# michaelriedl/2048-ppo-agent

Hardware: AMD Instinct MI355X
Metric: env-steps/sec at N parallel boards (full PPO loop: rollout with policy in the loop + GAE + update) (higher is better)
Workload: dtype u8 boards / bf16 policy; 1 GPU; 65536 parallel boards per GPU, Transformer policy bf16 (3.96 M params), full PPO iteration (BASELINE.json configs[2]; configs[3] when n_gpus=8); boards_per_gpu=65536, global_boards=65536, train_batch=2048, update_epochs=5, max_samples_per_epoch=300000, max_samples_per_epoch_is=global (each rank draws its 1/N share), as the reference's single subset, max_samples_per_epoch_per_rank=300000, rollout_mode=episodes (reference lock-step semantics), rng_mode=partitionable, parallelism=env-shard x1 + 1 grad all-reduce/minibatch

## Files before the change

2048-ppo-agent_amd/csrc/g2048_rowgemm.hip:

```cpp
#include <hip/hip_runtime.h>
#include <stdint.h>
#include <stdlib.h>

#include <type_traits>

#include "../../include/g2048.h"
#include "g2048_host.h"
#include "g2048_mfma.h"

namespace {

using namespace g2048_mfma;
using namespace g2048_host;

constexpr int RG_N = 256, RG_KC = 128, RG_THREADS = 512, RG_WAVES = 8;
template <int NB> struct RgShape {
    static constexpr int TT = 32 * NB, STAGE = TT * RG_KC * 2, PIECES = TT * (RG_KC / 8) / RG_THREADS, RPW = TT / RG_WAVES, BATCH = RPW / 2;
    static constexpr int LDS = 2 * STAGE + RG_WAVES * 3 * RG_N * 4 + RG_N * 4;
    static_assert(PIECES * RG_THREADS == TT * (RG_KC / 8) && RPW % 2 == 0 && BATCH >= 1, "tile shape");
};

enum { RG_FWD = 0, RG_BWD = 1 };

struct RowGemmArgs {
    const __bf16 *x;
    int64_t ldx;
    const __bf16 *w;
    int64_t w_tile_stride;
    const uint16_t *gh_extra;
    int extra_period;
    const float *bias;
    int64_t T;
    int K, tpw;
    const float *res;
    int64_t res_rs;
    const float *g_x;
    int g_x_period;
    const float *gamma, *beta;
    float *mean, *rstd;
    float *out_f32;
    uint16_t *out_bf16;
    float *partial;
    float eps, inv_keep;
    uint32_t thr, s0, s1;
    const uint64_t *seed_state;
};

template <int CTRL>
__device__ __forceinline__ float dpp_step(float v) {
    return v + __builtin_bit_cast(float, __builtin_amdgcn_update_dpp(0, __builtin_bit_cast(int, v), CTRL, 0xF, 0xF, true));
}
__device__ __forceinline__ float wave_sum_dpp(float v) {
    v = dpp_step<0xB1>(v);
    v = dpp_step<0x4E>(v);
    v = dpp_step<0x141>(v);
    v = dpp_step<0x140>(v);
    const int iv = __builtin_bit_cast(int, v);
    const float r0 = __builtin_bit_cast(float, __builtin_amdgcn_readlane(iv, 0)), r1 = __builtin_bit_cast(float, __builtin_amdgcn_readlane(iv, 16));
    const float r2 = __builtin_bit_cast(float, __builtin_amdgcn_readlane(iv, 32)), r3 = __builtin_bit_cast(float, __builtin_amdgcn_readlane(iv, 48));
    return (r0 + r1) + (r2 + r3);
}

template <int MODE, int NB, int NCH>
__global__ void __launch_bounds__(RG_THREADS, 2)
k_rowgemm(RowGemmArgs A) {
    constexpr int RG_NB = NB, RG_TT = RgShape<NB>::TT, RG_STAGE = RgShape<NB>::STAGE, RG_PIECES = RgShape<NB>::PIECES;
    constexpr int RG_RPW = RgShape<NB>::RPW, RG_BATCH = RgShape<NB>::BATCH;
    extern __shared__ __attribute__((aligned(16))) char smem[];
    const int tid = threadIdx.x, lane = tid & 63, r = lane & 31, h = lane >> 5;
    const int w = __builtin_amdgcn_readfirstlane(tid >> 6);
    float *const red = reinterpret_cast<float *>(smem + 2 * RG_STAGE);
    float *const bias_l = reinterpret_cast<float *>(smem + 2 * RG_STAGE + RG_WAVES * 3 * RG_N * 4);
    uint32_t s0 = A.s0, s1 = A.s1;
    mix_seed_state(A.seed_state, s0, s1);
    const int64_t n_tiles = (A.T + A.tpw - 1) / A.tpw;
    if (tid < RG_N) bias_l[tid] = (MODE == RG_FWD && A.bias) ? A.bias[tid] : 0.f;

    for (int64_t tile = blockIdx.x; tile < n_tiles; tile += gridDim.x) {
        const int64_t tok0 = tile * A.tpw;
        const int n_valid = (int)((A.T - tok0 < A.tpw) ? A.T - tok0 : A.tpw);
        uint32_t goff[RG_PIECES];
        const int row0 = tid >> 4, pc = tid & 15;
#pragma unroll
        for (int j = 0; j < RG_PIECES; ++j) {
            const int row = row0 + 32 * j;
            goff[j] = (uint32_t)((int64_t)(row < n_valid ? row : n_valid - 1) * A.ldx * 2) + 16u * (uint32_t)pc;
        }
        const uint32_t loff0 = (uint32_t)(row0 * (RG_KC * 2) + ((pc ^ (row0 & 15)) << 4));
        const char *const xg = reinterpret_cast<const char *>(A.x + tok0 * A.ldx);
        u32x4 G[3][RG_PIECES];
        unsigned kc = 0;
#define RG_GLOAD(P, ahead)                                                                                                \
    _Pragma("unroll") for (int j = 0; j < RG_PIECES; ++j) G[P][j] =                                                       \
        *reinterpret_cast<const u32x4 *>(xg + goff[j] + (size_t)(kc + (ahead)) * (RG_KC * 2))
#define RG_LSTORE(P, ST)                                                                                                  \
    _Pragma("unroll") for (int j = 0; j < RG_PIECES; ++j)                                                                 \
        *reinterpret_cast<u32x4 *>(smem + (ST) * RG_STAGE + loff0 + j * (32 * RG_KC * 2)) = G[P][j]
        constexpr int WR = 4, NG = 8 * NCH;
        const __bf16 *const wp = A.w + (size_t)w * A.w_tile_stride + lane * 8;
        bf16x8 W[WR];
        const uint32_t brow = (uint32_t)(r * (RG_KC * 2)), bx = (uint32_t)((h ^ (r & 15)) << 4);

        f32x16 acc[RG_NB];
        RG_GLOAD(0, 0);
        if constexpr (NCH > 1) { RG_GLOAD(1, 1); }
        if constexpr (NCH > 2) { RG_GLOAD(2, 2); }
#pragma unroll
        for (int g = 0; g < WR; ++g) W[g] = *reinterpret_cast<const bf16x8 *>(wp + (size_t)g * 512);
        lds_barrier();
#pragma unroll
        for (int b = 0; b < RG_NB; ++b) acc[b] = bias_tile(bias_l, 32 * w, h);
        RG_LSTORE(0, 0);
        lds_barrier();

        const bool norm = A.gamma != nullptr;
        const float4 gm = norm ? reinterpret_cast<const float4 *>(A.gamma)[lane] : make_float4(0.f, 0.f, 0.f, 0.f);
        auto row_tok = [&](int row) -> int64_t { return tok0 + (row < n_valid ? row : n_valid - 1); };
        constexpr bool PIPE = NB <= 3;
        constexpr int BB = RG_BATCH / 2, NBB = RG_RPW / BB;
        static_assert(RG_RPW % BB == 0, "backward batches");
        float4 fv[MODE == RG_FWD ? RG_RPW : 1];
        float4 bx0[2][MODE == RG_BWD ? BB : 1], bg0[2][MODE == RG_BWD ? BB : 1];
        float bmu[2][MODE == RG_BWD ? BB : 1], brs[2][MODE == RG_BWD ? BB : 1];
        auto bwd_load = [&](int k, auto parity) {
            constexpr int P = decltype(parity)::value;
#pragma unroll
            for (int j = 0; j < BB; ++j) {
                const int64_t tok = row_tok(w + RG_WAVES * (k * BB + j));
                bx0[P][j] = reinterpret_cast<const float4 *>(A.res + tok * A.res_rs)[lane];
                bmu[P][j] = A.mean[tok];
                brs[P][j] = A.rstd[tok];
                bg0[P][j] = make_float4(0.f, 0.f, 0.f, 0.f);
                if (A.g_x) {
                    if (A.g_x_period == 1) bg0[P][j] = reinterpret_cast<const float4 *>(A.g_x + tok * RG_N)[lane];
                    else if (tok % A.g_x_period == 0) bg0[P][j] = reinterpret_cast<const float4 *>(A.g_x + (tok / A.g_x_period) * RG_N)[lane];
                }
            }
        };
        auto fwd_load = [&](auto lo_c, auto hi_c) {
#pragma unroll
            for (int j = decltype(lo_c)::value; j < decltype(hi_c)::value; ++j)
                fv[j] = reinterpret_cast<const float4 *>(A.res + row_tok(w + RG_WAVES * j) * A.res_rs)[lane];
        };
        using I0 = std::integral_constant<int, 0>;
        using IB = std::integral_constant<int, RG_BATCH>;
        using IR = std::integral_constant<int, RG_RPW>;
#define RG_FRAG(st, s_) \
    *reinterpret_cast<const bf16x8 *>((st) + brow + ((32u * ((s_) / RG_NB)) ^ bx) + ((s_) % RG_NB) * (32 * RG_KC * 2))
#define RG_CHUNK(c)                                                                                                        \
    if constexpr ((c) < NCH) {                                                                                             \
        if constexpr ((c) == NCH - 1 && PIPE) {        \
            if (MODE == RG_FWD) fwd_load(I0{}, IB{});                                                                      \
            else bwd_load(0, I0{});                                                                                        \
        }                                                                                                                  \
        if constexpr ((c) + 3 < NCH) { RG_GLOAD((c) % 3, 3); }                                                             \
        const char *const st = smem + ((c) & 1) * RG_STAGE;                                                                \
        constexpr int PRE = 3, NS = 8 * RG_NB;     \
        bf16x8 q[PRE];                                                                                                     \
        _Pragma("unroll") for (int s_ = 0; s_ < PRE; ++s_) q[s_] = RG_FRAG(st, s_);                                        \
        _Pragma("unroll") for (int s_ = 0; s_ < NS; ++s_) {                                                                \
            __builtin_amdgcn_sched_barrier(0);                                                                             \
            const int ks = s_ / RG_NB, b = s_ % RG_NB, g = 8 * (c) + ks;                                                   \
            acc[b] = mfma(W[g % WR], q[s_ % PRE], acc[b]);                                                                 \
            if (s_ + PRE < NS) q[s_ % PRE] = RG_FRAG(st, s_ + PRE);                                                        \
            if (b == RG_NB - 1 && g + WR < NG) W[g % WR] = *reinterpret_cast<const bf16x8 *>(wp + (size_t)(kc * 8 + ks + WR) * 512); \
        }                                                                                                                  \
        __builtin_amdgcn_sched_barrier(0);                                                                                 \
        if constexpr ((c) + 1 < NCH) { RG_LSTORE(((c) + 1) % 3, ((c) + 1) & 1); }                                          \
        kc += 1;                                                                                                           \
        asm volatile("" : "+s"(kc));                                                                                       \
        lds_barrier();                                                                                                     \
    }
        RG_CHUNK(0) RG_CHUNK(1) RG_CHUNK(2) RG_CHUNK(3) RG_CHUNK(4) RG_CHUNK(5) RG_CHUNK(6) RG_CHUNK(7)
#undef RG_CHUNK
#undef RG_FRAG
#undef RG_GLOAD
#undef RG_LSTORE

#pragma unroll
        for (int b = 0; b < RG_NB; ++b) {
            const int trow = 32 * b + r;
#pragma unroll
            for (int g = 0; g < 4; ++g) {
                const uint32_t lo = f2bf(acc[b][4 * g + 0]) | (f2bf(acc[b][4 * g + 1]) << 16);
                const uint32_t hi = f2bf(acc[b][4 * g + 2]) | (f2bf(acc[b][4 * g + 3]) << 16);
                *reinterpret_cast<uint2 *>(smem + trow * 512 + (((4 * w + g) ^ (trow & 31)) << 4) + 8 * h) = make_uint2(lo, hi);
            }
        }
        lds_barrier();
        if (MODE == RG_FWD) {
            if (PIPE) fwd_load(IB{}, IR{});
            else fwd_load(I0{}, IR{});
        }
        auto tile_row = [&](int row) -> uint2 {
            return *reinterpret_cast<const uint2 *>(smem + row * 512 + ((((lane >> 1) ^ (row & 31))) << 4) + 8 * (lane & 1));
        };
        if (MODE == RG_FWD) {
            const float4 bt = norm ? reinterpret_cast<const float4 *>(A.beta)[lane] : make_float4(0.f, 0.f, 0.f, 0.f);
#pragma unroll
            for (int j0 = 0; j0 < RG_RPW; j0 += RG_BATCH) {
                if (w + RG_WAVES * j0 >= n_valid) break;
                float4 v[RG_BATCH];
                float s[RG_BATCH];
#pragma unroll
                for (int j = 0; j < RG_BATCH; ++j) {
                    const int row = w + RG_WAVES * (j0 + j), rowc = row < n_valid ? row : n_valid - 1;
                    const int64_t tok = tok0 + rowc;
                    const uint2 ab = tile_row(rowc);
                    float av[4] = {bf2f(ab.x & 0xFFFFu), bf2f(ab.x >> 16), bf2f(ab.y & 0xFFFFu), bf2f(ab.y >> 16)};
                    if (A.thr) {
                        const uint64_t base = (uint64_t)tok * RG_N + 4 * lane;
#pragma unroll
                        for (int q = 0; q < 4; ++q) av[q] = keep_elem(s0, s1, A.thr, base + q) ? av[q] * A.inv_keep : 0.0f;
                    }
                    v[j] = fv[j0 + j];
                    v[j].x += av[0]; v[j].y += av[1]; v[j].z += av[2]; v[j].w += av[3];
                    if (row < n_valid) reinterpret_cast<float4 *>(A.out_f32 + tok * RG_N)[lane] = v[j];
                    s[j] = v[j].x + v[j].y + v[j].z + v[j].w;
                }
#pragma unroll
                for (int j = 0; j < RG_BATCH; ++j) s[j] = wave_sum_dpp(s[j]);
                float mean[RG_BATCH];
#pragma unroll
                for (int j = 0; j < RG_BATCH; ++j) {
                    mean[j] = s[j] * (1.0f / RG_N);
                    v[j].x -= mean[j]; v[j].y -= mean[j]; v[j].z -= mean[j]; v[j].w -= mean[j];
                    s[j] = v[j].x * v[j].x + v[j].y * v[j].y + v[j].z * v[j].z + v[j].w * v[j].w;
                }
#pragma unroll
                for (int j = 0; j < RG_BATCH; ++j) s[j] = wave_sum_dpp(s[j]);
#pragma unroll
                for (int j = 0; j < RG_BATCH; ++j) {
                    const int row = w + RG_WAVES * (j0 + j);
                    const int64_t tok = tok0 + row;
                    const float rstd = rsqrtf(s[j] * (1.0f / RG_N) + A.eps);
                    const uint32_t lo = f2bf(v[j].x * rstd * gm.x + bt.x) | (f2bf(v[j].y * rstd * gm.y + bt.y) << 16);
                    const uint32_t hi = f2bf(v[j].z * rstd * gm.z + bt.z) | (f2bf(v[j].w * rstd * gm.w + bt.w) << 16);
                    if (row < n_valid) {
                        reinterpret_cast<uint2 *>(A.out_bf16 + tok * RG_N)[lane] = make_uint2(lo, hi);
                        if (lane == 0) {
                            A.mean[tok] = mean[j];
                            A.rstd[tok] = rstd;
                        }
                    }
                }
            }
        } else {
            float dg[4] = {0, 0, 0, 0}, db[4] = {0, 0, 0, 0}, dsum[4] = {0, 0, 0, 0};
            const float gg[4] = {gm.x, gm.y, gm.z, gm.w};
            auto bwd_batch = [&](int k, auto parity) {
                constexpr int P = decltype(parity)::value;
                if (PIPE && k + 1 < NBB && w + RG_WAVES * (k + 1) * BB < n_valid) bwd_load(k + 1, std::integral_constant<int, P ^ 1>{});
                float xh[BB][4], dxh[BB][4], c1[BB], c2[BB];
#pragma unroll
                for (int j = 0; j < BB; ++j) {
                    const int row = w + RG_WAVES * (k * BB + j), rowc = row < n_valid ? row : n_valid - 1;
                    const float ok = row < n_valid ? 1.f : 0.f;
                    const uint2 gb = tile_row(rowc);
                    float gh[4] = {bf2f(gb.x & 0xFFFFu), bf2f(gb.x >> 16), bf2f(gb.y & 0xFFFFu), bf2f(gb.y >> 16)};
                    if (A.gh_extra) {
                        const int64_t tk = tok0 + rowc;
                        if (tk % A.extra_period == 0) {
                            const uint2 eb = reinterpret_cast<const uint2 *>(A.gh_extra + (tk / A.extra_period) * RG_N)[lane];
                            gh[0] = bf2f(f2bf(gh[0] + bf2f(eb.x & 0xFFFFu))); gh[1] = bf2f(f2bf(gh[1] + bf2f(eb.x >> 16)));
                            gh[2] = bf2f(f2bf(gh[2] + bf2f(eb.y & 0xFFFFu))); gh[3] = bf2f(f2bf(gh[3] + bf2f(eb.y >> 16)));
                        }
                    }
                    const float xs[4] = {bx0[P][j].x, bx0[P][j].y, bx0[P][j].z, bx0[P][j].w};
                    c1[j] = c2[j] = 0.f;
#pragma unroll
                    for (int q = 0; q < 4; ++q) {
                        xh[j][q] = (xs[q] - bmu[P][j]) * brs[P][j];
                        dxh[j][q] = gh[q] * gg[q];
                        c1[j] += dxh[j][q];
                        c2[j] += dxh[j][q] * xh[j][q];
                        dg[q] += ok * (gh[q] * xh[j][q]);
                        db[q] += ok * gh[q];
                    }
                }
#pragma unroll
                for (int j = 0; j < BB; ++j) {
                    c1[j] = wave_sum_dpp(c1[j]);
                    c2[j] = wave_sum_dpp(c2[j]);
                }
#pragma unroll
                for (int j = 0; j < BB; ++j) {
                    const int row = w + RG_WAVES * (k * BB + j);
                    const bool ok = row < n_valid;
                    const int64_t tok = tok0 + (ok ? row : n_valid - 1);
                    float o[4] = {bg0[P][j].x, bg0[P][j].y, bg0[P][j].z, bg0[P][j].w};
                    const float m1 = c1[j] * (1.0f / RG_N), m2 = c2[j] * (1.0f / RG_N);
#pragma unroll
                    for (int q = 0; q < 4; ++q) o[q] += brs[P][j] * (dxh[j][q] - m1 - xh[j][q] * m2);
                    if (ok) reinterpret_cast<float4 *>(A.out_f32 + tok * RG_N)[lane] = make_float4(o[0], o[1], o[2], o[3]);
                    if (A.out_bf16) {
                        if (A.thr) {
                            const uint64_t base = (uint64_t)tok * RG_N + 4 * lane;
#pragma unroll
                            for (int q = 0; q < 4; ++q) o[q] = keep_elem(s0, s1, A.thr, base + q) ? o[q] * A.inv_keep : 0.0f;
                        }
                        uint32_t bq[4];
#pragma unroll
                        for (int q = 0; q < 4; ++q) {
                            bq[q] = f2bf(o[q]);
                            dsum[q] += ok ? bf2f(bq[q]) : 0.f;
                        }
                        if (ok) reinterpret_cast<uint2 *>(A.out_bf16 + tok * RG_N)[lane] = make_uint2(bq[0] | (bq[1] << 16), bq[2] | (bq[3] << 16));
                    }
                }
            };
            if (PIPE) {
#pragma unroll
                for (int k = 0; k < NBB; k += 2) {
                    if (w + RG_WAVES * k * BB < n_valid) bwd_batch(k, std::integral_constant<int, 0>{});
                    if (k + 1 < NBB && w + RG_WAVES * (k + 1) * BB < n_valid) bwd_batch(k + 1, std::integral_constant<int, 1>{});
                }
            } else {
#pragma unroll 1
                for (int k = 0; k < NBB; ++k) {
                    if (w + RG_WAVES * k * BB >= n_valid) break;
                    bwd_load(k, std::integral_constant<int, 0>{});
                    bwd_batch(k, std::integral_constant<int, 0>{});
                }
            }
#pragma unroll
            for (int q = 0; q < 4; ++q) {
                red[(w * 3 + 0) * RG_N + 4 * lane + q] = dg[q];
                red[(w * 3 + 1) * RG_N + 4 * lane + q] = db[q];
                red[(w * 3 + 2) * RG_N + 4 * lane + q] = dsum[q];
            }
            lds_barrier();
            for (int c = tid; c < 3 * RG_N; c += RG_THREADS) {
                float s = 0.f;
#pragma unroll
                for (int ww = 0; ww < RG_WAVES; ++ww) s += red[ww * 3 * RG_N + c];
                float *dst = A.partial + (int64_t)blockIdx.x * 3 * RG_N + c;
                *dst = (tile == (int64_t)blockIdx.x) ? s : *dst + s;
            }
        }
    }
}

inline int rg_tpw(int64_t T, int *nb) {
    const char *e = getenv("G2048_RG_TWO_TILES");
    const bool two = e && e[0] == '1';
    int64_t t = (T + 255) / 256;
    if (two) t = (T + 511) / 512;
    if (t <= 96 && (two || t <= 48)) {
        *nb = 3;
        return (int)(t < 32 ? 32 : t);
    }
    *nb = 5;
    return (int)(t > 160 ? 160 : t);
}

template <int MODE, int NB, int NCH>
int rg_launch3(RowGemmArgs &A, unsigned grid, hipStream_t stream) {
    const void *fn = reinterpret_cast<const void *>(k_rowgemm<MODE, NB, NCH>);
    constexpr int lds = RgShape<NB>::LDS;
    if (const int rc = allow_dynamic_lds(fn, lds)) return rc;
    hipLaunchKernelGGL((k_rowgemm<MODE, NB, NCH>), dim3(grid), dim3(RG_THREADS), lds, stream, A);
    return launch_status();
}
template <int MODE, int NB>
int rg_launch2(RowGemmArgs &A, unsigned grid, hipStream_t stream) {
    switch (A.K / RG_KC) {
        case 2: return rg_launch3<MODE, NB, 2>(A, grid, stream);
        case 4: return rg_launch3<MODE, NB, 4>(A, grid, stream);
        case 6: return rg_launch3<MODE, NB, 6>(A, grid, stream);
        case 8: return rg_launch3<MODE, NB, 8>(A, grid, stream);
        default: return G2048_EINVAL;
    }
}
template <int MODE>
int rg_launch(RowGemmArgs &A, hipStream_t stream) {
    int nb = 5;
    A.tpw = rg_tpw(A.T, &nb);
    const int64_t tiles = (A.T + A.tpw - 1) / A.tpw;
    const unsigned grid = (unsigned)(tiles < 256 ? tiles : 256);
    return nb == 3 ? rg_launch2<MODE, 3>(A, grid, stream) : rg_launch2<MODE, 5>(A, grid, stream);
}

inline bool rg_gemm_ok(const void *x, int64_t ldx, const void *w, int64_t T, int K) {
    return x && w && T > 0 && K >= 256 && K % 256 == 0 && K <= 1024 && ldx >= K && !(ldx & 7) && aligned16(x, w) &&
           (int64_t)160 * ldx * 2 < (1ll << 31);
}

}

extern "C" int64_t g2048_linear_add_ln_bwd_partial_rows(int64_t T) {
    if (T <= 0) return 0;
    int nb;
    const int tpw = rg_tpw(T, &nb);
    const int64_t tiles = (T + tpw - 1) / tpw;
    return tiles < 256 ? tiles : 256;
}

extern "C" int g2048_linear_add_ln_fwd(const void *u, int64_t ldu, const void *w_packed, const float *bias, int K, const float *x,
                                       int64_t x_row_stride, const float *gamma, const float *beta, float *x_new, void *h, float *mean,
                                       float *rstd, int64_t T, float eps, float p_drop, uint64_t seed, const uint64_t *seed_state,
                                       void *stream) {
    if (!rg_gemm_ok(u, ldu, w_packed, T, K) || !x || !gamma || !beta || !x_new || !h || !mean || !rstd || !(p_drop >= 0.f && p_drop < 1.f) ||
        (x_row_stride & 3) || !aligned16(x, gamma, beta, x_new, bias) ||
        ((uintptr_t)h & 7))
        return G2048_EINVAL;
    RowGemmArgs A{};
    A.x = (const __bf16 *)u; A.ldx = ldu; A.w = (const __bf16 *)w_packed; A.bias = bias; A.T = T; A.K = K;
    A.w_tile_stride = (int64_t)(K >> 4) * 512; A.extra_period = 1;
    A.res = x; A.res_rs = x_row_stride; A.gamma = gamma; A.beta = beta; A.mean = mean; A.rstd = rstd; A.out_f32 = x_new;
    A.out_bf16 = (uint16_t *)h; A.eps = eps; A.inv_keep = 1.0f / (1.0f - p_drop); A.thr = (uint32_t)(p_drop * 16777216.0f);
    A.s0 = (uint32_t)seed; A.s1 = (uint32_t)(seed >> 32); A.seed_state = seed_state; A.g_x_period = 1;
    return rg_launch<RG_FWD>(A, (hipStream_t)stream);
}

extern "C" int g2048_linear_add_ln_bwd(const void *dy, int64_t lddy, const void *wt_packed, int64_t wt_tile_stride, int K,
                                       const float *x_norm, int64_t x_row_stride, const float *g_x, int g_x_period, const void *g_h_extra,
                                       int extra_period, const float *mean, const float *rstd, const float *gamma, float *dx, void *da,
                                       float *partial, int64_t T, float p_drop, uint64_t seed, const uint64_t *seed_state, void *stream) {
    if (wt_tile_stride == 0) wt_tile_stride = (int64_t)(K >> 4) * 512;
    if (wt_tile_stride < (int64_t)(K >> 4) * 512 || (wt_tile_stride & 7) || (g_h_extra && extra_period < 1) || ((uintptr_t)g_h_extra & 7))
        return G2048_EINVAL;
    if (!rg_gemm_ok(dy, lddy, wt_packed, T, K) || !x_norm || !mean || !rstd || !gamma || !dx || !partial || g_x_period < 1 ||
        !(p_drop >= 0.f && p_drop < 1.f) || (x_row_stride & 3) ||
        !aligned16(x_norm, g_x, gamma, dx) || ((uintptr_t)da & 7) || ((uintptr_t)partial & 3))
        return G2048_EINVAL;
    if ((g_x && T % g_x_period != 0) || (g_h_extra && T % extra_period != 0)) return G2048_EINVAL;
    RowGemmArgs A{};
    A.x = (const __bf16 *)dy; A.ldx = lddy; A.w = (const __bf16 *)wt_packed; A.T = T; A.K = K;
    A.w_tile_stride = wt_tile_stride; A.gh_extra = (const uint16_t *)g_h_extra; A.extra_period = extra_period < 1 ? 1 : extra_period;
    A.res = x_norm; A.res_rs = x_row_stride; A.g_x = g_x; A.g_x_period = g_x_period; A.gamma = gamma;
    A.mean = const_cast<float *>(mean); A.rstd = const_cast<float *>(rstd); A.out_f32 = dx; A.out_bf16 = (uint16_t *)da;
    A.partial = partial; A.inv_keep = 1.0f / (1.0f - p_drop); A.thr = da ? (uint32_t)(p_drop * 16777216.0f) : 0u;
    A.s0 = (uint32_t)seed; A.s1 = (uint32_t)(seed >> 32); A.seed_state = seed_state;
    return rg_launch<RG_BWD>(A, (hipStream_t)stream);
}
```

Baseline: 3.939 million env-steps/sec.

## Use buffer loads and split residual-row prefetch in row-GEMM LN kernel

Replaces global pointer loads of activations, weights and residual rows with raw buffer loads through per-tile resource descriptors, which gives scalar offsets and hardware bounds clamping. In the backward pass, mean/rstd and periodic g_x offsets are loaded once per lane and broadcast with readlane instead of per-row scalar loads. For larger NB in forward mode, residual-row and gamma prefetches are split into two requests issued inside the MFMA loop so their latency hides behind compute. It also adds optional timestamp instrumentation and an env-selected serial fallback, plus stride validation, which raise code complexity and register pressure.

```diff
diff --git a/2048-ppo-agent_amd/csrc/g2048_rowgemm.hip b/2048-ppo-agent_amd/csrc/g2048_rowgemm.hip
--- a/2048-ppo-agent_amd/csrc/g2048_rowgemm.hip
+++ b/2048-ppo-agent_amd/csrc/g2048_rowgemm.hip
@@ -61,24 +61,59 @@
     return (r0 + r1) + (r2 + r3);
 }
 
-template <int MODE, int NB, int NCH>
+typedef __amdgpu_buffer_rsrc_t rsrc_t;
+__device__ __forceinline__ rsrc_t rg_rsrc(const void *p, uint32_t bytes) {
+    return __builtin_amdgcn_make_buffer_rsrc(const_cast<void *>(p), 0, (int)bytes, 0x00020000);
+}
+template <class V>
+__device__ __forceinline__ V rg_load16(rsrc_t rs, uint32_t lane_off, uint32_t scalar_off) {
+    return __builtin_bit_cast(V, __builtin_amdgcn_raw_buffer_load_b128(rs, (int)lane_off, (int)scalar_off, 0));
+}
+
+#ifdef G2048_RG_STAMPS
+constexpr int RG_PHASES = 8;
+__device__ unsigned long long g_rg_stamps[2][RG_PHASES];
+struct RgStampSite {
+    __device__ __forceinline__ static bool on(int lane, int w) { return lane == 0 && (w == 0 || w == 7) && blockIdx.x % 16 == 0; }
+    __device__ __forceinline__ static unsigned long long *table(int w) { return g_rg_stamps[w == 0 ? 0 : 1]; }
+};
+#define RG_STAMP(k) stamps.mark(k)
+#define RG_TOUCH(v) asm volatile("" ::"v"(v))
+#define RG_DRAIN() asm volatile("s_waitcnt vmcnt(0)" ::: "memory")
+#else
+#define RG_STAMP(k)
+#define RG_TOUCH(v)
+#define RG_DRAIN()
+#endif
+enum { RG_PH_FIRST_CHUNK, RG_PH_KLOOP, RG_PH_STAGE, RG_PH_WAIT_FIRST, RG_PH_ROWS, RG_PH_WAIT_LATER, RG_PH_DRAIN, RG_PH_PARTIAL };
+
+template <int MODE, int NB, int NCH, bool SERIAL>
 __global__ void __launch_bounds__(RG_THREADS, 2)
 k_rowgemm(RowGemmArgs A) {
     constexpr int RG_NB = NB, RG_TT = RgShape<NB>::TT, RG_STAGE = RgShape<NB>::STAGE, RG_PIECES = RgShape<NB>::PIECES;
     constexpr int RG_RPW = RgShape<NB>::RPW, RG_BATCH = RgShape<NB>::BATCH;
     extern __shared__ __attribute__((aligned(16))) char smem[];
-    const int tid = threadIdx.x, lane = tid & 63, r = lane & 31, h = lane >> 5;
-    const int w = __builtin_amdgcn_readfirstlane(tid >> 6);
+    const int tid0 = threadIdx.x;
+    const int w = __builtin_amdgcn_readfirstlane(tid0 >> 6);
     float *const red = reinterpret_cast<float *>(smem + 2 * RG_STAGE);
     float *const bias_l = reinterpret_cast<float *>(smem + 2 * RG_STAGE + RG_WAVES * 3 * RG_N * 4);
     uint32_t s0 = A.s0, s1 = A.s1;
     mix_seed_state(A.seed_state, s0, s1);
     const int64_t n_tiles = (A.T + A.tpw - 1) / A.tpw;
-    if (tid < RG_N) bias_l[tid] = (MODE == RG_FWD && A.bias) ? A.bias[tid] : 0.f;
+    if (tid0 < RG_N) bias_l[tid0] = (MODE == RG_FWD && A.bias) ? A.bias[tid0] : 0.f;
+#ifdef G2048_RG_STAMPS
+    Stamps<RG_PHASES, RgStampSite> stamps;
+    stamps.start();
+#endif
+    const uint32_t res_rs4 = (uint32_t)(A.res_rs * 4);
 
     for (int64_t tile = blockIdx.x; tile < n_tiles; tile += gridDim.x) {
         const int64_t tok0 = tile * A.tpw;
         const int n_valid = (int)((A.T - tok0 < A.tpw) ? A.T - tok0 : A.tpw);
+        int tid = tid0;
+        asm volatile("" : "+v"(tid));
+        const int lane = tid & 63, r = lane & 31, h = lane >> 5;
+        const uint32_t l16 = 16u * (uint32_t)lane;
         uint32_t goff[RG_PIECES];
         const int row0 = tid >> 4, pc = tid & 15;
 #pragma unroll
@@ -87,17 +122,39 @@
             goff[j] = (uint32_t)((int64_t)(row < n_valid ? row : n_valid - 1) * A.ldx * 2) + 16u * (uint32_t)pc;
         }
         const uint32_t loff0 = (uint32_t)(row0 * (RG_KC * 2) + ((pc ^ (row0 & 15)) << 4));
-        const char *const xg = reinterpret_cast<const char *>(A.x + tok0 * A.ldx);
+        const rsrc_t xr = rg_rsrc(A.x + tok0 * A.ldx, (uint32_t)(((int64_t)(n_valid - 1) * A.ldx + A.K) * 2));
+        const rsrc_t wr = rg_rsrc(A.w + (size_t)w * A.w_tile_stride, (uint32_t)(A.K >> 4) * 1024u);
+        const rsrc_t rr = rg_rsrc(A.res + tok0 * A.res_rs, (uint32_t)(((int64_t)(n_valid - 1) * A.res_rs + RG_N) * 4));
+        constexpr uint32_t RG_NONE = 0xFFFFFFFFu;
+        float vmu = 0.f, vrs = 0.f;
+        uint32_t vgo = RG_NONE, veo = RG_NONE;
+        rsrc_t gxr = rg_rsrc(A.res, 0), exr = rg_rsrc(A.res, 0);
+        const rsrc_t nullr = rg_rsrc(A.res, 0);
+        if (MODE == RG_BWD) {
+            const int mrow = w + RG_WAVES * (lane < RgShape<NB>::RPW ? lane : 0);
+            const uint32_t mrowc = (uint32_t)(mrow < n_valid ? mrow : n_valid - 1);
+            vmu = A.mean[tok0 + mrowc];
+            vrs = A.rstd[tok0 + mrowc];
+            auto periodic = [&](const void *base, int period, uint32_t row_bytes, uint32_t &voff) -> rsrc_t {
+                if (!base) return nullr;
+                const uint32_t per = (uint32_t)period, m0 = (uint32_t)(tok0 % period), q0 = m0 ? 1u : 0u;
+                const uint32_t rows = (m0 + (uint32_t)n_valid - 1u) / per + 1u - q0;
+                const uint32_t t = m0 + mrowc, q = t / per;
+                voff = t == q * per ? (q - q0) * row_bytes : RG_NONE;
+                return rg_rsrc(reinterpret_cast<const char *>(base) + (tok0 / period + q0) * row_bytes, rows * row_bytes);
+            };
+            gxr = periodic(A.g_x, A.g_x_period, RG_N * 4, vgo);
+            exr = periodic(A.gh_extra, A.extra_period, RG_N * 2, veo);
+        }
+        auto row_lane = [&](uint32_t v, int idx) -> uint32_t { return (uint32_t)__builtin_amdgcn_readlane((int)v, idx); };
         u32x4 G[3][RG_PIECES];
         unsigned kc = 0;
 #define RG_GLOAD(P, ahead)                                                                                                \
-    _Pragma("unroll") for (int j = 0; j < RG_PIECES; ++j) G[P][j] =                                                       \
-        *reinterpret_cast<const u32x4 *>(xg + goff[j] + (size_t)(kc + (ahead)) * (RG_KC * 2))
+    _Pragma("unroll") for (int j = 0; j < RG_PIECES; ++j) G[P][j] = rg_load16<u32x4>(xr, goff[j], (kc + (ahead)) * (RG_KC * 2))
 #define RG_LSTORE(P, ST)                                                                                                  \
     _Pragma("unroll") for (int j = 0; j < RG_PIECES; ++j)                                                                 \
         *reinterpret_cast<u32x4 *>(smem + (ST) * RG_STAGE + loff0 + j * (32 * RG_KC * 2)) = G[P][j]
         constexpr int WR = 4, NG = 8 * NCH;
-        const __bf16 *const wp = A.w + (size_t)w * A.w_tile_stride + lane * 8;
         bf16x8 W[WR];
         const uint32_t brow = (uint32_t)(r * (RG_KC * 2)), bx = (uint32_t)((h ^ (r & 15)) << 4);
 
@@ -106,53 +163,53 @@
         if constexpr (NCH > 1) { RG_GLOAD(1, 1); }
         if constexpr (NCH > 2) { RG_GLOAD(2, 2); }
 #pragma unroll
-        for (int g = 0; g < WR; ++g) W[g] = *reinterpret_cast<const bf16x8 *>(wp + (size_t)g * 512);
+        for (int g = 0; g < WR; ++g) W[g] = rg_load16<bf16x8>(wr, l16, g * 1024u);
         lds_barrier();
 #pragma unroll
         for (int b = 0; b < RG_NB; ++b) acc[b] = bias_tile(bias_l, 32 * w, h);
         RG_LSTORE(0, 0);
         lds_barrier();
+        RG_STAMP(RG_PH_FIRST_CHUNK);
 
         const bool norm = A.gamma != nullptr;
-        const float4 gm = norm ? reinterpret_cast<const float4 *>(A.gamma)[lane] : make_float4(0.f, 0.f, 0.f, 0.f);
-        auto row_tok = [&](int row) -> int64_t { return tok0 + (row < n_valid ? row : n_valid - 1); };
-        constexpr bool PIPE = NB <= 3;
+        constexpr bool GM_LATE = NB > 3 && !SERIAL && MODE == RG_FWD;
+        float4 gm = make_float4(0.f, 0.f, 0.f, 0.f);
+        if (!GM_LATE && norm) gm = reinterpret_cast<const float4 *>(A.gamma)[lane];
+        constexpr bool PIPE = NB <= 3 || (!SERIAL && MODE == RG_FWD);
+        constexpr bool TWO_REQ = NB > 3 && PIPE;
+        constexpr int ROWREQ = NB <= 3 ? -1 : 4 * NB - 1, REQ_C0 = NCH >= 2 ? NCH - 2 : 0;
         constexpr int BB = RG_BATCH / 2, NBB = RG_RPW / BB;
         static_assert(RG_RPW % BB == 0, "backward batches");
-        float4 fv[MODE == RG_FWD ? RG_RPW : 1];
-        float4 bx0[2][MODE == RG_BWD ? BB : 1], bg0[2][MODE == RG_BWD ? BB : 1];
-        float bmu[2][MODE == RG_BWD ? BB : 1], brs[2][MODE == RG_BWD ? BB : 1];
+        f32x4 fv[MODE == RG_FWD ? RG_RPW : 1];
+        f32x4 bx0[2][MODE == RG_BWD ? BB : 1], bg0[2][MODE == RG_BWD ? BB : 1];
         auto bwd_load = [&](int k, auto parity) {
             constexpr int P = decltype(parity)::value;
 #pragma unroll
             for (int j = 0; j < BB; ++j) {
-                const int64_t tok = row_tok(w + RG_WAVES * (k * BB + j));
-                bx0[P][j] = reinterpret_cast<const float4 *>(A.res + tok * A.res_rs)[lane];
-                bmu[P][j] = A.mean[tok];
-                brs[P][j] = A.rstd[tok];
-                bg0[P][j] = make_float4(0.f, 0.f, 0.f, 0.f);
-                if (A.g_x) {
-                    if (A.g_x_period == 1) bg0[P][j] = reinterpret_cast<const float4 *>(A.g_x + tok * RG_N)[lane];
-                    else if (tok % A.g_x_period == 0) bg0[P][j] = reinterpret_cast<const float4 *>(A.g_x + (tok / A.g_x_period) * RG_N)[lane];
-                }
+                const int row = w + RG_WAVES * (k * BB + j);
+                const uint32_t rowc = (uint32_t)(row < n_valid ? row : n_valid - 1);
+                bx0[P][j] = rg_load16<f32x4>(rr, l16, rowc * res_rs4);
+                const uint32_t go = row_lane(vgo, k * BB + j);
+                bg0[P][j] = rg_load16<f32x4>(go != RG_NONE ? gxr : nullr, l16, go != RG_NONE ? go : 0u);
             }
         };
         auto fwd_load = [&](auto lo_c, auto hi_c) {
 #pragma unroll
-            for (int j = decltype(lo_c)::value; j < decltype(hi_c)::value; ++j)
-                fv[j] = reinterpret_cast<const float4 *>(A.res + row_tok(w + RG_WAVES * j) * A.res_rs)[lane];
+            for (int j = decltype(lo_c)::value; j < decltype(hi_c)::value; ++j) {
+                const int row = w + RG_WAVES * j;
+                fv[j] = rg_load16<f32x4>(rr, l16, (uint32_t)(row < n_valid ? row : n_valid - 1) * res_rs4);
+            }
         };
-        using I0 = std::integral_constant<int, 0>;
-        using IB = std::integral_constant<int, RG_BATCH>;
-        using IR = std::integral_constant<int, RG_RPW>;
+        auto first_rows = [&]() {
+            if (GM_LATE && norm) gm = __builtin_bit_cast(float4, rg_load16<f32x4>(rg_rsrc(A.gamma, RG_N * 4), l16, 0u));
+            if (MODE == RG_FWD) fwd_load(std::integral_constant<int, 0>{}, std::integral_constant<int, RG_BATCH>{});
+            else bwd_load(0, std::integral_constant<int, 0>{});
+        };
 #define RG_FRAG(st, s_) \
     *reinterpret_cast<const bf16x8 *>((st) + brow + ((32u * ((s_) / RG_NB)) ^ bx) + ((s_) % RG_NB) * (32 * RG_KC * 2))
 #define RG_CHUNK(c)                                                                                                        \
     if constexpr ((c) < NCH) {                                                                                             \
-        if constexpr ((c) == NCH - 1 && PIPE) {        \
-            if (MODE == RG_FWD) fwd_load(I0{}, IB{});                                                                      \
-            else bwd_load(0, I0{});                                                                                        \
-        }                                                                                                                  \
+        if constexpr ((c) == NCH - 1 && PIPE && ROWREQ < 0) { first_rows(); }            \
         if constexpr ((c) + 3 < NCH) { RG_GLOAD((c) % 3, 3); }                                                             \
         const char *const st = smem + ((c) & 1) * RG_STAGE;                                                                \
         constexpr int PRE = 3, NS = 8 * RG_NB;     \
@@ -163,7 +220,10 @@
             const int ks = s_ / RG_NB, b = s_ % RG_NB, g = 8 * (c) + ks;                                                   \
             acc[b] = mfma(W[g % WR], q[s_ % PRE], acc[b]);                                                                 \
             if (s_ + PRE < NS) q[s_ % PRE] = RG_FRAG(st, s_ + PRE);                                                        \
-            if (b == RG_NB - 1 && g + WR < NG) W[g % WR] = *reinterpret_cast<const bf16x8 *>(wp + (size_t)(kc * 8 + ks + WR) * 512); \
+            if (b == RG_NB - 1 && g + WR < NG) W[g % WR] = rg_load16<bf16x8>(wr, l16, (kc * 8 + ks + WR) * 1024u);         \
+            if (TWO_REQ && (c) == REQ_C0 && s_ == ROWREQ) first_rows();                                                    \
+            if (TWO_REQ && (c) == NCH - 1 && s_ == ROWREQ)                                                                 \
+                fwd_load(std::integral_constant<int, RG_BATCH>{}, std::integral_constant<int, RG_RPW>{});                  \
         }                                                                                                                  \
         __builtin_amdgcn_sched_barrier(0);                                                                                 \
         if constexpr ((c) + 1 < NCH) { RG_LSTORE(((c) + 1) % 3, ((c) + 1) & 1); }                                          \
@@ -172,6 +232,7 @@
         lds_barrier();                                                                                                     \
     }
         RG_CHUNK(0) RG_CHUNK(1) RG_CHUNK(2) RG_CHUNK(3) RG_CHUNK(4) RG_CHUNK(5) RG_CHUNK(6) RG_CHUNK(7)
+        RG_STAMP(RG_PH_KLOOP);
 #undef RG_CHUNK
 #undef RG_FRAG
 #undef RG_GLOAD
@@ -188,34 +249,42 @@
             }
         }
         lds_barrier();
+        RG_STAMP(RG_PH_STAGE);
         if (MODE == RG_FWD) {
-            if (PIPE) fwd_load(IB{}, IR{});
-            else fwd_load(I0{}, IR{});
+            if (!TWO_REQ) fwd_load(std::integral_constant<int, PIPE ? RG_BATCH : 0>{}, std::integral_constant<int, RG_RPW>{});
+            RG_TOUCH(fv[RG_BATCH - 1].w);
+            RG_STAMP(RG_PH_WAIT_FIRST);
         }
+        int le = lane, we = w;
+        asm volatile("" : "+v"(le), "+s"(we));
         auto tile_row = [&](int row) -> uint2 {
-            return *reinterpret_cast<const uint2 *>(smem + row * 512 + ((((lane >> 1) ^ (row & 31))) << 4) + 8 * (lane & 1));
+            return *reinterpret_cast<const uint2 *>(smem + row * 512 + ((((le >> 1) ^ (row & 31))) << 4) + 8 * (le & 1));
         };
         if (MODE == RG_FWD) {
-            const float4 bt = norm ? reinterpret_cast<const float4 *>(A.beta)[lane] : make_float4(0.f, 0.f, 0.f, 0.f);
+            const float4 bt = norm ? reinterpret_cast<const float4 *>(A.beta)[le] : make_float4(0.f, 0.f, 0.f, 0.f);
 #pragma unroll
             for (int j0 = 0; j0 < RG_RPW; j0 += RG_BATCH) {
-                if (w + RG_WAVES * j0 >= n_valid) break;
-                float4 v[RG_BATCH];
+                if (we + RG_WAVES * j0 >= n_valid) break;
+                if (j0 > 0) {
+                    RG_TOUCH(fv[RG_RPW - 1].w);
+                    RG_STAMP(RG_PH_WAIT_LATER);
+                }
+                f32x4 v[RG_BATCH];
                 float s[RG_BATCH];
 #pragma unroll
                 for (int j = 0; j < RG_BATCH; ++j) {
-                    const int row = w + RG_WAVES * (j0 + j), rowc = row < n_valid ? row : n_valid - 1;
+                    const int row = we + RG_WAVES * (j0 + j), rowc = row < n_valid ? row : n_valid - 1;
                     const int64_t tok = tok0 + rowc;
                     const uint2 ab = tile_row(rowc);
                     float av[4] = {bf2f(ab.x & 0xFFFFu), bf2f(ab.x >> 16), bf2f(ab.y & 0xFFFFu), bf2f(ab.y >> 16)};
                     if (A.thr) {
-                        const uint64_t base = (uint64_t)tok * RG_N + 4 * lane;
+                        const uint64_t base = (uint64_t)tok * RG_N + 4 * le;
 #pragma unroll
                         for (int q = 0; q < 4; ++q) av[q] = keep_elem(s0, s1, A.thr, base + q) ? av[q] * A.inv_keep : 0.0f;
                     }
                     v[j] = fv[j0 + j];
                     v[j].x += av[0]; v[j].y += av[1]; v[j].z += av[2]; v[j].w += av[3];
-                    if (row < n_valid) reinterpret_cast<float4 *>(A.out_f32 + tok * RG_N)[lane] = v[j];
+                    if (row < n_valid) reinterpret_cast<f32x4 *>(A.out_f32 + tok * RG_N)[le] = v[j];
                     s[j] = v[j].x + v[j].y + v[j].z + v[j].w;
                 }
 #pragma unroll
@@ -231,46 +300,54 @@
                 for (int j = 0; j < RG_BATCH; ++j) s[j] = wave_sum_dpp(s[j]);
 #pragma unroll
                 for (int j = 0; j < RG_BATCH; ++j) {
-                    const int row = w + RG_WAVES * (j0 + j);
+                    const int row = we + RG_WAVES * (j0 + j);
                     const int64_t tok = tok0 + row;
                     const float rstd = rsqrtf(s[j] * (1.0f / RG_N) + A.eps);
                     const uint32_t lo = f2bf(v[j].x * rstd * gm.x + bt.x) | (f2bf(v[j].y * rstd * gm.y + bt.y) << 16);
                     const uint32_t hi = f2bf(v[j].z * rstd * gm.z + bt.z) | (f2bf(v[j].w * rstd * gm.w + bt.w) << 16);
                     if (row < n_valid) {
-                        reinterpret_cast<uint2 *>(A.out_bf16 + tok * RG_N)[lane] = make_uint2(lo, hi);
-                        if (lane == 0) {
+                        reinterpret_cast<uint2 *>(A.out_bf16 + tok * RG_N)[le] = make_uint2(lo, hi);
+                        if (le == 0) {
                             A.mean[tok] = mean[j];
                             A.rstd[tok] = rstd;
                         }
                     }
                 }
-            }
+                RG_STAMP(RG_PH_ROWS);
+            }
+            RG_DRAIN();
+            RG_STAMP(RG_PH_DRAIN);
         } else {
             float dg[4] = {0, 0, 0, 0}, db[4] = {0, 0, 0, 0}, dsum[4] = {0, 0, 0, 0};
             const float gg[4] = {gm.x, gm.y, gm.z, gm.w};
             auto bwd_batch = [&](int k, auto parity) {
                 constexpr int P = decltype(parity)::value;
-                if (PIPE && k + 1 < NBB && w + RG_WAVES * (k + 1) * BB < n_valid) bwd_load(k + 1, std::integral_constant<int, P ^ 1>{});
-                float xh[BB][4], dxh[BB][4], c1[BB], c2[BB];
+                if (PIPE && k + 1 < NBB && we + RG_WAVES * (k + 1) * BB < n_valid) bwd_load(k + 1, std::integral_constant<int, P ^ 1>{});
+                RG_TOUCH(bx0[P][BB - 1].w);
+                RG_TOUCH(bg0[P][BB - 1].w);
+                RG_STAMP(k == 0 ? RG_PH_WAIT_FIRST : RG_PH_WAIT_LATER);
+                float xh[BB][4], dxh[BB][4], c1[BB], c2[BB], mu[BB], rs[BB];
 #pragma unroll
                 for (int j = 0; j < BB; ++j) {
-                    const int row = w + RG_WAVES * (k * BB + j), rowc = row < n_valid ? row : n_valid - 1;
+                    const int row = we + RG_WAVES * (k * BB + j), rowc = row < n_valid ? row : n_valid - 1;
                     const float ok = row < n_valid ? 1.f : 0.f;
                     const uint2 gb = tile_row(rowc);
                     float gh[4] = {bf2f(gb.x & 0xFFFFu), bf2f(gb.x >> 16), bf2f(gb.y & 0xFFFFu), bf2f(gb.y >> 16)};
                     if (A.gh_extra) {
-                        const int64_t tk = tok0 + rowc;
-                        if (tk % A.extra_period == 0) {
-                            const uint2 eb = reinterpret_cast<const uint2 *>(A.gh_extra + (tk / A.extra_period) * RG_N)[lane];
+                        const uint32_t eo = row_lane(veo, k * BB + j);
+                        if (eo != RG_NONE) {
+                            const uint2 eb = __builtin_bit_cast(uint2, __builtin_amdgcn_raw_buffer_load_b64(exr, (int)(8u * (uint32_t)le), (int)eo, 0));
                             gh[0] = bf2f(f2bf(gh[0] + bf2f(eb.x & 0xFFFFu))); gh[1] = bf2f(f2bf(gh[1] + bf2f(eb.x >> 16)));
                             gh[2] = bf2f(f2bf(gh[2] + bf2f(eb.y & 0xFFFFu))); gh[3] = bf2f(f2bf(gh[3] + bf2f(eb.y >> 16)));
                         }
                     }
                     const float xs[4] = {bx0[P][j].x, bx0[P][j].y, bx0[P][j].z, bx0[P][j].w};
                     c1[j] = c2[j] = 0.f;
+                    mu[j] = __builtin_bit_cast(float, row_lane(__builtin_bit_cast(uint32_t, vmu), k * BB + j));
+                    rs[j] = __builtin_bit_cast(float, row_lane(__builtin_bit_cast(uint32_t, vrs), k * BB + j));
 #pragma unroll
                     for (int q = 0; q < 4; ++q) {
-                        xh[j][q] = (xs[q] - bmu[P][j]) * brs[P][j];
+                        xh[j][q] = (xs[q] - mu[j]) * rs[j];
                         dxh[j][q] = gh[q] * gg[q];
                         c1[j] += dxh[j][q];
                         c2[j] += dxh[j][q] * xh[j][q];
@@ -285,17 +362,17 @@
                 }
 #pragma unroll
                 for (int j = 0; j < BB; ++j) {
-                    const int row = w + RG_WAVES * (k * BB + j);
+                    const int row = we + RG_WAVES * (k * BB + j);
                     const bool ok = row < n_valid;
                     const int64_t tok = tok0 + (ok ? row : n_valid - 1);
                     float o[4] = {bg0[P][j].x, bg0[P][j].y, bg0[P][j].z, bg0[P][j].w};
                     const float m1 = c1[j] * (1.0f / RG_N), m2 = c2[j] * (1.0f / RG_N);
 #pragma unroll
-                    for (int q = 0; q < 4; ++q) o[q] += brs[P][j] * (dxh[j][q] - m1 - xh[j][q] * m2);
-                    if (ok) reinterpret_cast<float4 *>(A.out_f32 + tok * RG_N)[lane] = make_float4(o[0], o[1], o[2], o[3]);
+                    for (int q = 0; q < 4; ++q) o[q] += rs[j] * (dxh[j][q] - m1 - xh[j][q] * m2);
+                    if (ok) reinterpret_cast<float4 *>(A.out_f32 + tok * RG_N)[le] = make_float4(o[0], o[1], o[2], o[3]);
                     if (A.out_bf16) {
                         if (A.thr) {
-                            const uint64_t base = (uint64_t)tok * RG_N + 4 * lane;
+                            const uint64_t base = (uint64_t)tok * RG_N + 4 * le;
 #pragma unroll
                             for (int q = 0; q < 4; ++q) o[q] = keep_elem(s0, s1, A.thr, base + q) ? o[q] * A.inv_keep : 0.0f;
                         }
@@ -305,40 +382,52 @@
                             bq[q] = f2bf(o[q]);
                             dsum[q] += ok ? bf2f(bq[q]) : 0.f;
                         }
-                        if (ok) reinterpret_cast<uint2 *>(A.out_bf16 + tok * RG_N)[lane] = make_uint2(bq[0] | (bq[1] << 16), bq[2] | (bq[3] << 16));
+                        if (ok) reinterpret_cast<uint2 *>(A.out_bf16 + tok * RG_N)[le] = make_uint2(bq[0] | (bq[1] << 16), bq[2] | (bq[3] << 16));
                     }
                 }
+                RG_STAMP(RG_PH_ROWS);
             };
             if (PIPE) {
 #pragma unroll
                 for (int k = 0; k < NBB; k += 2) {
-                    if (w + RG_WAVES * k * BB < n_valid) bwd_batch(k, std::integral_constant<int, 0>{});
-                    if (k + 1 < NBB && w + RG_WAVES * (k + 1) * BB < n_valid) bwd_batch(k + 1, std::integral_constant<int, 1>{});
+                    if (we + RG_WAVES * k * BB < n_valid) bwd_batch(k, std::integral_constant<int, 0>{});
+                    if (k + 1 < NBB && we + RG_WAVES * (k + 1) * BB < n_valid) bwd_batch(k + 1, std::integral_constant<int, 1>{});
                 }
             } else {
 #pragma unroll 1
                 for (int k = 0; k < NBB; ++k) {
-                    if (w + RG_WAVES * k * BB >= n_valid) break;
+                    if (we + RG_WAVES * k * BB >= n_valid) break;
                     bwd_load(k, std::integral_constant<int, 0>{});
                     bwd_batch(k, std::integral_constant<int, 0>{});
                 }
             }
+            RG_DRAIN();
+            RG_STAMP(RG_PH_DRAIN);
 #pragma unroll
             for (int q = 0; q < 4; ++q) {
-                red[(w * 3 + 0) * RG_N + 4 * lane + q] = dg[q];
-                red[(w * 3 + 1) * RG_N + 4 * lane + q] = db[q];
-                red[(w * 3 + 2) * RG_N + 4 * lane + q] = dsum[q];
+                red[(we * 3 + 0) * RG_N + 4 * le + q] = dg[q];
+                red[(we * 3 + 1) * RG_N + 4 * le + q] = db[q];
+                red[(we * 3 + 2) * RG_N + 4 * le + q] = dsum[q];
             }
             lds_barrier();
-            for (int c = tid; c < 3 * RG_N; c += RG_THREADS) {
+            for (int c = 64 * we + le; c < 3 * RG_N; c += RG_THREADS) {
                 float s = 0.f;
 #pragma unroll
                 for (int ww = 0; ww < RG_WAVES; ++ww) s += red[ww * 3 * RG_N + c];
                 float *dst = A.partial + (int64_t)blockIdx.x * 3 * RG_N + c;
                 *dst = (tile == (int64_t)blockIdx.x) ? s : *dst + s;
             }
+            RG_STAMP(RG_PH_PARTIAL);
         }
     }
+#ifdef G2048_RG_STAMPS
+    stamps.flush(tid0 & 63, w);
+#endif
+}
+
+inline bool rg_serial_rows() {
+    const char *e = getenv("G2048_RG_SERIAL_ROWS");
+    return e && e[0] == '1';
 }
 
 inline int rg_tpw(int64_t T, int *nb) {
@@ -354,13 +443,19 @@
     return (int)(t > 160 ? 160 : t);
 }
 
+template <int MODE, int NB, int NCH, bool SERIAL>
+int rg_launch4(RowGemmArgs &A, unsigned grid, hipStream_t stream) {
+    const void *fn = reinterpret_cast<const void *>(k_rowgemm<MODE, NB, NCH, SERIAL>);
+    constexpr int lds = RgShape<NB>::LDS;
+    if (const int rc = allow_dynamic_lds(fn, lds)) return rc;
+    hipLaunchKernelGGL((k_rowgemm<MODE, NB, NCH, SERIAL>), dim3(grid), dim3(RG_THREADS), lds, stream, A);
+    return launch_status();
+}
 template <int MODE, int NB, int NCH>
 int rg_launch3(RowGemmArgs &A, unsigned grid, hipStream_t stream) {
-    const void *fn = reinterpret_cast<const void *>(k_rowgemm<MODE, NB, NCH>);
-    constexpr int lds = RgShape<NB>::LDS;
-    if (const int rc = allow_dynamic_lds(fn, lds)) return rc;
-    hipLaunchKernelGGL((k_rowgemm<MODE, NB, NCH>), dim3(grid), dim3(RG_THREADS), lds, stream, A);
-    return launch_status();
+    constexpr bool HAS_ARM = NB > 3 && MODE == RG_FWD;
+    if (HAS_ARM && rg_serial_rows()) return rg_launch4<MODE, NB, NCH, HAS_ARM>(A, grid, stream);
+    return rg_launch4<MODE, NB, NCH, false>(A, grid, stream);
 }
 template <int MODE, int NB>
 int rg_launch2(RowGemmArgs &A, unsigned grid, hipStream_t stream) {
@@ -385,6 +480,7 @@
     return x && w && T > 0 && K >= 256 && K % 256 == 0 && K <= 1024 && ldx >= K && !(ldx & 7) && aligned16(x, w) &&
            (int64_t)160 * ldx * 2 < (1ll << 31);
 }
+inline bool rg_res_ok(int64_t row_stride) { return row_stride >= RG_N && (int64_t)160 * row_stride * 4 < (1ll << 31); }
 
 }
 
@@ -401,7 +497,7 @@
                                        float *rstd, int64_t T, float eps, float p_drop, uint64_t seed, const uint64_t *seed_state,
                                        void *stream) {
     if (!rg_gemm_ok(u, ldu, w_packed, T, K) || !x || !gamma || !beta || !x_new || !h || !mean || !rstd || !(p_drop >= 0.f && p_drop < 1.f) ||
-        (x_row_stride & 3) || !aligned16(x, gamma, beta, x_new, bias) ||
+        (x_row_stride & 3) || !rg_res_ok(x_row_stride) || !aligned16(x, gamma, beta, x_new, bias) ||
         ((uintptr_t)h & 7))
         return G2048_EINVAL;
     RowGemmArgs A{};
@@ -421,7 +517,7 @@
     if (wt_tile_stride < (int64_t)(K >> 4) * 512 || (wt_tile_stride & 7) || (g_h_extra && extra_period < 1) || ((uintptr_t)g_h_extra & 7))
         return G2048_EINVAL;
     if (!rg_gemm_ok(dy, lddy, wt_packed, T, K) || !x_norm || !mean || !rstd || !gamma || !dx || !partial || g_x_period < 1 ||
-        !(p_drop >= 0.f && p_drop < 1.f) || (x_row_stride & 3) ||
+        !(p_drop >= 0.f && p_drop < 1.f) || (x_row_stride & 3) || !rg_res_ok(x_row_stride) ||
         !aligned16(x_norm, g_x, gamma, dx) || ((uintptr_t)da & 7) || ((uintptr_t)partial & 3))
         return G2048_EINVAL;
     if ((g_x && T % g_x_period != 0) || (g_h_extra && T % extra_period != 0)) return G2048_EINVAL;
@@ -434,3 +530,14 @@
     A.s0 = (uint32_t)seed; A.s1 = (uint32_t)(seed >> 32); A.seed_state = seed_state;
     return rg_launch<RG_BWD>(A, (hipStream_t)stream);
 }
+
+#ifdef G2048_RG_STAMPS
+extern "C" int g2048_debug_rg_stamps(unsigned long long *out , int reset) {
+    if (hipMemcpyFromSymbol(out, HIP_SYMBOL(g_rg_stamps), sizeof(g_rg_stamps)) != hipSuccess) return -1;
+    if (reset) {
+        static const unsigned long long zero[2][RG_PHASES] = {};
+        if (hipMemcpyToSymbol(HIP_SYMBOL(g_rg_stamps), zero, sizeof(zero)) != hipSuccess) return -1;
+    }
+    return 0;
+}
+#endif
```

Measured after the change: 3.953 million env-steps/sec, median of 6. About the same (+0.4%).
